# xarray-contrib/xeofs

Hardware: AMD Instinct MI355X
Metric: EOF randomized-SVD GB/s (algorithmic: 16 passes x n x p x 4 B per fit / fit time) (higher is better)
Workload: dtype f32 data, split-fp16 MFMA (f16x3+f16x3), f32 accumulate

## Files before the change

xeofs_amd/csrc/eofx_abi.hip:

```cpp
#include <chrono>
#include "eofx_hfft.hpp"
#include "eofx_kernels.hpp"
#include "eofx_fit.hpp"
#include "eofx_gram.hpp"
#include "eofx_axb_dma.hpp"
#include "eofx_hosteig.hpp"
#include "eofx_lag.hpp"
#include "eofx_gw.hpp"
#include "eofx_spca.hpp"
#include "eofx_lagcov.hpp"
#ifndef EOFX_AXB_DMA_DEFAULT
#define EOFX_AXB_DMA_DEFAULT 1
#endif

#if !defined(__HIP_DEVICE_COMPILE__)
#include <immintrin.h>
#endif
#include <algorithm>
#include <array>
#include <atomic>
#include <cmath>
#include <complex>
#include <cstdarg>
#include <cstdio>
// ... 880 lines not shown
        hipLaunchKernelGGL((axb_f16_dma_kernel<2, 0, true>), dim3(gx, 1), dim3(256), 0, ctx->stream, raw, ld, (int)rows, cols, aff,
                           aff_ld, ctx->axb_planes, pairs_all, out, L, rows_pad, K, plan.kps, plan.S, rt, nfull * 64, a_scale, bmax, act);
      else
        hipLaunchKernelGGL((axb_f16_dma_kernel<2, 0, false>), dim3(gx, 1), dim3(256), 0, ctx->stream, raw, ld, (int)rows, cols, aff,
                           aff_ld, ctx->axb_planes, pairs_all, out, L, rows_pad, K, plan.kps, plan.S, rt, nfull * 64, a_scale, bmax,
                           (const int*)nullptr);
      KCHK();
    }
  } else if (nfull > 0) {
    if (masked)
      hipLaunchKernelGGL((axb_f16_kernel<4, 0, true>), dim3(gx, nfull), dim3(256), 0, ctx->stream, raw, ld, (int)rows, cols, aff, aff_ld, Y,
                         L, out, L, rows_pad, K, plan.kps, plan.S, rt, 0, a_scale, bmax, act);
    else
      hipLaunchKernelGGL(axb_f16_kernel<4>, dim3(gx, nfull), dim3(256), 0, ctx->stream, raw, ld, (int)rows, cols, aff, aff_ld, Y, L, out,
                         L, rows_pad, K, plan.kps, plan.S, rt, 0, a_scale, bmax);
    KCHK();
  }
  if (!dma && rem) {
    if (masked)
      hipLaunchKernelGGL((axb_f16_kernel<2, 0, true>), dim3(gx, 1), dim3(256), 0, ctx->stream, raw, ld, (int)rows, cols, aff, aff_ld, Y, L,
                         out, L, rows_pad, K, plan.kps, plan.S, rt, nfull * 64, a_scale, bmax, act);
    else
      hipLaunchKernelGGL(axb_f16_kernel<2>, dim3(gx, 1), dim3(256), 0, ctx->stream, raw, ld, (int)rows, cols, aff, aff_ld, Y, L, out,
                         L, rows_pad, K, plan.kps, plan.S, rt, nfull * 64, a_scale, bmax);
    KCHK();
  }
  if (ctx->profile) {
    HIPCHK(hipEventRecord(ev1, ctx->stream));
    ctx->prof_events.emplace_back(ev0, ev1, 1);
    ctx->prof_flops += 2.0 * (double)K * (double)rows_pad * (double)L;
    ctx->prof_bytes += (double)K * (double)rows * 4.0 * (nfull + (rem ? 1 : 0));
  }
  if (plan.S > 1) {
    const int64_t count4 = rows_pad * L / 4;
    hipLaunchKernelGGL(splitk_reduce_kernel, dim3((int)std::min<int64_t>((count4 + 255) / 256, amax_out ? 2048 : 4096)), dim3(256), 0,
                       ctx->stream, out, W, count4, plan.S, amax_out);
    KCHK();
  }
  return EOFX_OK;
}

static int gram_parts(int64_t rows, int L) {
  const int64_t by_rows = std::min<int64_t>((rows + 127) / 128, 256);
  const int64_t by_mem = ((int64_t)128 << 20) / ((int64_t)L * L * 8);
  if (const char* ev = std::getenv("EOFX_GRAM_PARTS")) return std::max(1, atoi(ev));
  return (int)std::max<int64_t>(1, std::min(by_rows, std::max<int64_t>(by_mem, 1)));
}

static int launch_gram(eofx_ctx* ctx, const float* P, int64_t rows, int L, double* G) {
  const int nb = (L + 63) / 64;
  const int nbx = gram_parts(rows, L);
  ArenaScope scope(ctx);
  ARENA(double, part, (size_t)nbx * L * L);
  hipLaunchKernelGGL(gram_mfma_kernel, dim3(nbx, nb * nb), dim3(256), 0, ctx->stream, P, rows, L, part);
  KCHK();
  const int64_t count = (int64_t)L * L;
  hipLaunchKernelGGL(f64_reduce_kernel, dim3((int)((count + 63) / 64)), dim3(256), 0, ctx->stream,
                     part, G, count, nbx);
  KCHK();
  return EOFX_OK;
}
static int launch_matmul(eofx_ctx* ctx, const float* P, int64_t rows, int L, const double* Mx, int Lo,
                         float* out, bool upper = false) {
  int KW = (int)std::min<int64_t>(round_up(L, 64), 256);
  if (L > 256) {
    static const int kw_env = std::getenv("EOFX_PMM_KW") ? atoi(std::getenv("EOFX_PMM_KW")) : 0;
    if (kw_env == 128 || kw_env == 256) KW = kw_env;
  }
  const size_t smem = (size_t)KW * PMM_LD * sizeof(double);
  if (smem > 64 * 1024)
    HIPCHK(hipFuncSetAttribute(reinterpret_cast<const void*>(panel_matmul_kernel<false>), hipFuncAttributeMaxDynamicSharedMemorySize, (int)smem));
  const int64_t units = (rows + 127) / 128;
  const int64_t gx = L <= KW ? std::min<int64_t>(units, 1024) : units;
  dim3 grid((int)std::max<int64_t>(1, gx), (Lo + 63) / 64);
  hipLaunchKernelGGL(panel_matmul_kernel<false>, grid, dim3(256), smem, ctx->stream, P, rows, L, Mx, Lo, out, KW, amax_new(ctx, out),
                     (int64_t)0, (int64_t)0, 1, (const float*)nullptr, upper ? 1 : 0);
  KCHK();
  return EOFX_OK;
}
static int launch_matmul_gen(eofx_ctx* ctx, const float* P, int64_t ldp, int64_t slab, int cpb, int64_t rows, int L, const double* Mx, int Lo,
                             const float* sub, float* out) {
  const int KW = (int)std::min<int64_t>(round_up(L, 64), 256);
  const size_t smem = (size_t)KW * PMM_LD * sizeof(double);
  if (smem > 64 * 1024)
    HIPCHK(hipFuncSetAttribute(reinterpret_cast<const void*>(panel_matmul_kernel<true>), hipFuncAttributeMaxDynamicSharedMemorySize, (int)smem));
  const int64_t units = (rows + 127) / 128;
  const int64_t gx = L <= KW ? std::min<int64_t>(units, 1024) : units;
  dim3 grid((int)std::max<int64_t>(1, gx), (Lo + 63) / 64);
  hipLaunchKernelGGL(panel_matmul_kernel<true>, grid, dim3(256), smem, ctx->stream, P, rows, L, Mx, Lo, out, KW, amax_new(ctx, out), ldp,
                     slab, cpb, sub);
  KCHK();
  return EOFX_OK;
}
static int launch_xgram(eofx_ctx* ctx, const float* Pa, int64_t lda, int La, const float* Pb, int64_t ldb, int Lb, int64_t rows, double* C) {
  const int nbx = (int)std::max<int64_t>(1, std::min<int64_t>((rows + 127) / 128, std::max<int64_t>(1, ((int64_t)32 << 20) / ((int64_t)La * Lb * 8))));
  ArenaScope scope(ctx);
  ARENA(double, part, (size_t)nbx * La * Lb);
  hipLaunchKernelGGL(xgram_mfma_kernel, dim3(nbx, (La / 64) * (Lb / 64)), dim3(256), 0, ctx->stream, Pa, lda, Pb, ldb, rows, La, Lb, part);
  KCHK();
  const int64_t count = (int64_t)La * Lb;
  hipLaunchKernelGGL(f64_reduce_kernel, dim3((int)((count + 63) / 64)), dim3(256), 0, ctx->stream, part, C, count, nbx);
  KCHK();
  return EOFX_OK;
}

static void host_chol_rinv(const double* G, int L, int l, double* Rinv, double tol) {
  std::vector<double> A((size_t)l * l, 0.0), X((size_t)l * l, 0.0), d0(l);
// ... 9 lines not shown
    const double rjj = dj ? 1.0 : std::sqrt(d);
    const double piv = dj ? 0.0 : 1.0 / rjj;
    A[(size_t)j * l + j] = rjj;
    double* rowj = &A[(size_t)j * l];
    for (int c = j + 1; c < l; ++c) rowj[c] *= piv;
    for (int r = j + 1; r < l; ++r) {
      const double f = rowj[r];
      if (f == 0.0) continue;
      double* rowr = &A[(size_t)r * l];
      for (int c = r; c < l; ++c) rowr[c] -= f * rowj[c];
    }
  }
  for (int c = 0; c < l; ++c) {
    if (dead[c]) continue;
    X[(size_t)c * l + c] = 1.0 / A[(size_t)c * l + c];
    for (int r = c - 1; r >= 0; --r) {
      double sum = 0.0;
      for (int t = r + 1; t <= c; ++t) sum += A[(size_t)r * l + t] * X[(size_t)t * l + c];
      X[(size_t)r * l + c] = -sum / A[(size_t)r * l + r];
    }
  }
  for (int r = 0; r < L; ++r)
    for (int c = 0; c < L; ++c) Rinv[(size_t)r * L + c] = (r < l && c < l) ? X[(size_t)r * l + c] : 0.0;
}

static int launch_rinv(eofx_ctx* ctx, const double* G, int L, int l, double* Rinv);
static size_t rinv_blocked_bytes(int l);
static bool matmul_nt_ok(int64_t rows, int L, int Lo);
static size_t matmul_nt_scratch(eofx_ctx* ctx, int64_t rows, int L, int Lo);
static int launch_matmul_nt(eofx_ctx* ctx, const float* P, int64_t rows, int L, const double* Mx, int Lo, float* out);
static int launch_cholqr(eofx_ctx* ctx, const float* P, int64_t rows, int L, int l, const double* G,
                         float* out) {
  ArenaScope scope(ctx);
  ARENA(double, Rinv, (size_t)L * L);
  CHK(launch_rinv(ctx, G, L, l, Rinv));
  return launch_matmul(ctx, P, rows, L, Rinv, L, out, true);
}

static int launch_colminmax(eofx_ctx* ctx, const float* P, int64_t rows, int L, float* mx, float* mn) {
  const int nparts = (int)std::max<int64_t>(1, std::min<int64_t>((rows + 127) / 128, 1024));
  ArenaScope scope(ctx);
  ARENA(float, pmx, (size_t)nparts * L);
  ARENA(float, pmn, (size_t)nparts * L);
  hipLaunchKernelGGL(colminmax_part_kernel, dim3(nparts, (L + 63) / 64), dim3(256), 0, ctx->stream, P,
                     rows, L, pmx, pmn);
  KCHK();
  hipLaunchKernelGGL(colminmax_final_kernel, dim3((L + 63) / 64), dim3(256), 0, ctx->stream, pmx, pmn,
                     nparts, L, mx, mn);
  KCHK();
  return EOFX_OK;
}

static int export_panel(eofx_ctx* ctx, const float* P, int64_t rows, int L, int k, const double* sign,
                        float* dst) {
  if (!dst) return EOFX_OK;
  ArenaScope scope(ctx);
  double* dsign = nullptr;
  if (sign) {
    dsign = arena_alloc<double>(ctx, k);
    if (!dsign) return set_err(ctx, EOFX_ERR_NOMEM, "arena exhausted (export sign)");
    CHK(copy_in(ctx, dsign, sign, sizeof(double) * k));
  }
  float* tmp = dst;
  const bool dev = is_device_ptr(dst);
  if (!dev) {
    tmp = arena_alloc<float>(ctx, (size_t)rows * k);
    if (!tmp) return set_err(ctx, EOFX_ERR_NOMEM, "arena exhausted (export staging)");
  }
  const int64_t total = rows * k;
  const int blocks = (int)std::min<int64_t>((total + 255) / 256, 8192);
  hipLaunchKernelGGL(panel_export_kernel, dim3(blocks), dim3(256), 0, ctx->stream, P, rows, L, k, dsign,
                     tmp);
  KCHK();
  if (!dev) {
    CHK(copy_out(ctx, dst, tmp, sizeof(float) * total));
    HIPCHK(hipStreamSynchronize(ctx->stream));
  }
  return EOFX_OK;
}

static int import_panel(eofx_ctx* ctx, const float* src, int64_t rows, int l, float* P, int64_t rows_pad,
                        int L) {
  ArenaScope scope(ctx);
  const float* dsrc = src;
  if (!is_device_ptr(src)) {
    float* tmp = arena_alloc<float>(ctx, (size_t)rows * l);
    if (!tmp) return set_err(ctx, EOFX_ERR_NOMEM, "arena exhausted (import staging)");
    CHK(copy_in(ctx, tmp, src, sizeof(float) * rows * l));
    dsrc = tmp;
  }
  const int64_t total = rows_pad * (L / 4);
  const int blocks = (int)std::min<int64_t>((total + 255) / 256, 2048);
  hipLaunchKernelGGL(panel_import_kernel, dim3(blocks), dim3(256), 0, ctx->stream, dsrc, rows, l, P,
                     rows_pad, L, amax_new(ctx, P));
  KCHK();
  if (dsrc != src) HIPCHK(hipStreamSynchronize(ctx->stream));
  return EOFX_OK;
}

static void* pool_take(eofx_ctx* ctx, size_t bytes) {
  for (size_t i = 0; i < ctx->pool.size(); ++i)
    if (ctx->pool[i].second == bytes) {
      void* p = ctx->pool[i].first;
      ctx->pool_bytes -= bytes;
      ctx->pool.erase(ctx->pool.begin() + i);
      return p;
    }
  return nullptr;
}
static void pool_trim(eofx_ctx* ctx) {
  if (ctx->pool.empty()) return;
// ... 912 lines not shown
        int64_t off = 0;
        for (size_t i = 0; i < npairs; ++i) {
          const int m1 = 64 * seg[2 * i], m2 = 64 * seg[2 * i + 1];
          merge(off, m1, m2, 1, 0);
          KCHK();
          off += m1 + m2;
          next.push_back(seg[2 * i] + seg[2 * i + 1]);
        }
      }
      if (seg.size() & 1) next.push_back(seg.back());
      seg.swap(next);
    }
  }
  hipLaunchKernelGGL(chol_blocked_export_kernel, dim3(512), dim3(256), 0, ctx->stream, (const double*)X, Lb, l, Rinv, L);
  KCHK();
  return EOFX_OK;
}
static int launch_rinv(eofx_ctx* ctx, const double* G, int L, int l, double* Rinv) {
  if (l <= 64) {
    hipLaunchKernelGGL(chol_rinv_kernel, dim3(1), dim3(256), 0, ctx->stream, G, L, l, Rinv, 1e-13, (const double*)nullptr);
    KCHK();
  } else if (ctx->arena_size - ctx->arena_off >= rinv_blocked_bytes(l) && !std::getenv("EOFX_HOST_RINV")) {
    CHK(launch_rinv_blocked(ctx, G, L, l, Rinv));
  } else {
    std::vector<double> hG((size_t)L * L), hR((size_t)L * L);
    HIPCHK(hipMemcpyAsync(hG.data(), G, sizeof(double) * L * L, hipMemcpyDeviceToHost, ctx->stream));
    HIPCHK(hipStreamSynchronize(ctx->stream));
    host_chol_rinv(hG.data(), L, l, hR.data(), 1e-13);
    HIPCHK(hipMemcpyAsync(Rinv, hR.data(), sizeof(double) * L * L, hipMemcpyHostToDevice, ctx->stream));
    HIPCHK(hipStreamSynchronize(ctx->stream));
  }
  return EOFX_OK;
}

constexpr int EOFX_FIT_FALLBACK = 1;
typedef std::function<int(const float*, float*, int)> FirstFwd;
typedef std::function<int(const float*, float*, int)> RangeFinder;
static int rsvd_core(eofx_ctx* ctx, const LinOp& op, int k, int l, int n_iter, const float* omega,
                     RsvdOut& out, const FirstFwd* first_fwd = nullptr, const RangeFinder* range = nullptr) {
  const int L = (int)round_up(l, 32);
  const int Lo = (int)round_up(k, 32);
  AmaxScope amax_scope(ctx);
  ARENA(float, Zs, (size_t)op.small_pad * L);
  ARENA(float, Ws, (size_t)op.small_pad * L);
  ARENA(float, Yt, (size_t)op.tall_pad * L);
  ARENA(float, Qt, (size_t)op.tall_pad * L);
  ARENA(float, Tv, (size_t)op.tall_pad * Lo);
  ARENA(float, Sv, (size_t)op.small_pad * Lo);
  ARENA(double, G, (size_t)L * L);
  ARENA(double, G0, (size_t)L * L);
  ARENA(double, R2, (size_t)L * L);
  ARENA(double, Md, (size_t)L * Lo);
  ARENA(double, Md2, (size_t)L * Lo);
  double* pin = nullptr;
  CHK(pinned_scratch(ctx, &pin));
  if ((size_t)2 * L * L > EOFX_PINNED_DOUBLES) return set_err(ctx, EOFX_ERR_ARG, "internal: sketch too wide for the host scratch");

  CHK(import_panel(ctx, omega, op.small, l, Zs, op.small_pad, L));
  bool first_done = false;
  auto fwd = [&](const float* z, float* y, int prec) -> int {
    if (first_fwd && !first_done) {
      first_done = true;
      return (*first_fwd)(z, y, L);
    }
    first_done = true;
    return op.fwd(z, y, L, prec);
  };
  auto gram_tall = [&](const float* Pn, double* Gout) -> int {
    CHK(launch_gram(ctx, Pn, op.tall_pad, L, Gout));
    return op.reduce_tall_gram ? op.reduce_tall_gram(Gout, (int64_t)L * L) : EOFX_OK;
  };
  auto gram_small = [&](const float* Pn, double* Gout) -> int {
    CHK(launch_gram(ctx, Pn, op.small_pad, L, Gout));
    return op.reduce_small_gram ? op.reduce_small_gram(Gout, (int64_t)L * L) : EOFX_OK;
  };
  const int pp = ctx->prec_power, pf = ctx->prec_final;
  const bool orth_always = orth_tall_rule(op.rule_tall_pad > 0 ? op.rule_tall_pad : op.tall_pad, L, pp);
  bool orth_rest = orth_always;
  hipEvent_t peaked_ev = nullptr;
  bool peaked_pending = false;
  int rc = EOFX_OK;
  for (int it = 0; it < (range ? 0 : n_iter) && rc == EOFX_OK; ++it) {
    rc = fwd(Zs, Yt, pp);
    if (rc != EOFX_OK) break;
    if (peaked_pending) {
      peaked_pending = false;
      if (hipEventSynchronize(peaked_ev) != hipSuccess) rc = set_err(ctx, EOFX_ERR_HIP, "event wait failed");
      else orth_rest = eofx_peaked_spectrum(pin, L, l) != 0;
      if (rc != EOFX_OK) break;
    }
    if (it == 0 || orth_rest) {
      if ((rc = gram_tall(Yt, G)) != EOFX_OK) break;
      if ((rc = launch_cholqr(ctx, Yt, op.tall_pad, L, l, G, Qt)) != EOFX_OK) break;
      rc = op.bwd(Qt, Ws, L, pp);
    } else {
      rc = op.bwd(Yt, Ws, L, pp);
    }
    if (rc != EOFX_OK) break;
    const bool ask = it == 0 && !orth_always && n_iter > 1;
    if ((rc = gram_small(Ws, ask ? G0 : G)) != EOFX_OK) break;
    if (ask) {
      if (hipMemcpyAsync(pin, G0, sizeof(double) * L * L, hipMemcpyDeviceToHost, ctx->stream) != hipSuccess ||
          (!peaked_ev && hipEventCreateWithFlags(&peaked_ev, hipEventDisableTiming) != hipSuccess) ||
          hipEventRecord(peaked_ev, ctx->stream) != hipSuccess) {
        rc = set_err(ctx, EOFX_ERR_HIP, "asynchronous Gram download failed");
        break;
      }
      peaked_pending = true;
    }
    rc = launch_cholqr(ctx, Ws, op.small_pad, L, l, ask ? G0 : G, Zs);
  }
  if (peaked_ev) {
    if (peaked_pending) (void)hipEventSynchronize(peaked_ev);
    (void)hipEventDestroy(peaked_ev);
  }
  if (rc != EOFX_OK) return rc;
  if (range) CHK((*range)(Zs, Yt, L));
  else CHK(fwd(Zs, Yt, pp));
  CHK(gram_tall(Yt, G));
  CHK(launch_cholqr(ctx, Yt, op.tall_pad, L, l, G, Qt));
  CHK(gram_tall(Qt, G));
  CHK(launch_rinv(ctx, G, L, l, R2));
  CHK(op.bwd(Qt, Zs, L, pf));
  CHK(launch_matmul(ctx, Zs, op.small_pad, L, R2, L, Ws));
  CHK(gram_small(Ws, G));
  double* hG = pin;
  double* hR2 = pin + (size_t)L * L;
  HIPCHK(hipMemcpyAsync(hG, G, sizeof(double) * L * L, hipMemcpyDeviceToHost, ctx->stream));
  HIPCHK(hipMemcpyAsync(hR2, R2, sizeof(double) * L * L, hipMemcpyDeviceToHost, ctx->stream));
  HIPCHK(hipStreamSynchronize(ctx->stream));
  std::vector<double> Gl((size_t)l * l), w(l), Uh((size_t)l * l);
  for (int i = 0; i < l; ++i)
    for (int j = 0; j < l; ++j) {
      const double v = 0.5 * (hG[(size_t)i * L + j] + hG[(size_t)j * L + i]);
      if (!std::isfinite(v))
        return set_err(ctx, EOFX_ERR_LINALG,
                       "SVD failed. This may be due to isolated NaN values in the data.");
      Gl[(size_t)i * l + j] = v;
    }
  eofx_host_eigh_f64(Gl.data(), l, w.data(), Uh.data());
  out.s.assign(k, 0.0);
  std::vector<double> M1((size_t)L * Lo, 0.0), M2((size_t)L * Lo, 0.0);
  std::vector<double> invs(k);
  for (int j = 0; j < k; ++j) {
    const double sv = std::sqrt(std::max(w[j], 0.0));
    out.s[j] = sv;
    invs[j] = sv > 0.0 ? 1.0 / sv : 0.0;
  }
  for (int i = 0; i < l; ++i) {
    double* m1 = &M1[(size_t)i * Lo];
    for (int q = 0; q < l; ++q) {
      const double r = hR2[(size_t)i * L + q];
      const double* uq = &Uh[(size_t)q * l];
      for (int j = 0; j < k; ++j) m1[j] += r * uq[j];
    }
    for (int j = 0; j < k; ++j) M2[(size_t)i * Lo + j] = Uh[(size_t)i * l + j] * invs[j];
  }
  HIPCHK(hipMemcpyAsync(Md, M1.data(), sizeof(double) * L * Lo, hipMemcpyHostToDevice, ctx->stream));
  HIPCHK(hipMemcpyAsync(Md2, M2.data(), sizeof(double) * L * Lo, hipMemcpyHostToDevice, ctx->stream));
  CHK(launch_matmul(ctx, Qt, op.tall_pad, L, Md, Lo, Tv));
  CHK(launch_matmul(ctx, Ws, op.small_pad, L, Md2, Lo, Sv));
  HIPCHK(hipStreamSynchronize(ctx->stream));
  out.Tvec = Tv;
  out.Svec = Sv;
  out.Lo = Lo;
  out.tall_pad = op.tall_pad;
  out.small_pad = op.small_pad;
  return EOFX_OK;
}

static size_t rsvd_scratch_bytes(int64_t tall_pad, int64_t small_pad, int l, int k) {
  const size_t L = (size_t)round_up(l, 32), Lo = (size_t)round_up(k, 32);
  size_t b = 0;
  b += 2 * small_pad * L * 4 + 2 * tall_pad * L * 4 + tall_pad * Lo * 4 + small_pad * Lo * 4;
  b += atb_scratch_bytes(small_pad, tall_pad, (int)L);
  b += atb_scratch_bytes(tall_pad, small_pad, (int)L);
  b += atb_scratch_bytes(small_pad, tall_pad, (int)Lo);
  b += (size_t)(4 * gram_parts(std::max(tall_pad, small_pad), (int)L) + 8) * L * L * 8 + 2 * L * Lo * 8 + 4096;
  b += (size_t)std::max(tall_pad, small_pad) * (Lo + L) * 4;
  if (l > 64) b += rinv_blocked_bytes(l);
  b += 4 << 20;
  return b;
}

static int comm_allreduce(eofx_ctx* ctx, void* buf, int64_t count, int dtype, int op);
static int sign_rule(eofx_ctx* ctx, const float* Vpanel, int64_t rows, int Lo, int k,
                     std::vector<double>& sign, bool over_ranks = false) {
  ArenaScope scope(ctx);
  ARENA(float, mx, 2 * (size_t)Lo);
  float* mn = mx + Lo;
  CHK(launch_colminmax(ctx, Vpanel, rows, Lo, mx, mn));
  if (over_ranks) {
    hipLaunchKernelGGL(negate_kernel, dim3(1), dim3(256), 0, ctx->stream, mn, Lo);
    KCHK();
    CHK(comm_allreduce(ctx, mx, 2 * (int64_t)Lo, 0, 1));
    hipLaunchKernelGGL(negate_kernel, dim3(1), dim3(256), 0, ctx->stream, mn, Lo);
    KCHK();
  }
  std::vector<float> hmx(Lo), hmn(Lo);
  HIPCHK(hipMemcpyAsync(hmx.data(), mx, sizeof(float) * Lo, hipMemcpyDeviceToHost, ctx->stream));
  HIPCHK(hipMemcpyAsync(hmn.data(), mn, sizeof(float) * Lo, hipMemcpyDeviceToHost, ctx->stream));
  HIPCHK(hipStreamSynchronize(ctx->stream));
  sign.assign(k, 1.0);
  for (int j = 0; j < k; ++j) sign[j] = (std::fabs(hmx[j]) >= std::fabs(hmn[j])) ? 1.0 : -1.0;
  return EOFX_OK;
}

typedef std::function<int(double*, int64_t)> GramReduce;
static int fix_null_columns(eofx_ctx* ctx, float* P, int64_t rows, int64_t rows_pad, int Lo, int k, int first,
                            const GramReduce* reduce = nullptr, int64_t rows_total = -1) {
  if (rows_total < 0) rows_total = rows;
  if (first >= k || rows_total <= first) return EOFX_OK;
  if (!reduce) {
    const size_t need = (size_t)rows_pad * Lo * 4 + (size_t)(gram_parts(rows_pad, Lo) + 4) * Lo * Lo * 8 + (64 << 10);
    if (ctx->arena_size - ctx->arena_off < need) return EOFX_OK;
  }
  ArenaScope scope(ctx);
  ARENA(double, G, (size_t)Lo * Lo);
  ARENA(double, Mx, (size_t)Lo * Lo);
  ARENA(float, tmp, (size_t)rows_pad * Lo);
  ARENA(int, dflag, Lo);
  const int m = k - first;
  std::vector<double> hG((size_t)Lo * Lo), hM((size_t)Lo * Lo);
  std::vector<int> flag(Lo, 0);
  const int blocks = (int)std::max<int64_t>(1, std::min<int64_t>((rows + 255) / 256, 4096));
  auto gram = [&]() -> int {
    CHK(launch_gram(ctx, P, rows_pad, Lo, G));
    if (reduce && *reduce) CHK((*reduce)(G, (int64_t)Lo * Lo));
    HIPCHK(hipMemcpyAsync(hG.data(), G, sizeof(double) * Lo * Lo, hipMemcpyDeviceToHost, ctx->stream));
    HIPCHK(hipStreamSynchronize(ctx->stream));
    return EOFX_OK;
// ... 47 lines not shown
      }
    }
    if (dependent) {
      if (rounds_done > 0) break;
      CHK(refill());
      continue;
    }
    for (int c = 0; c < m; ++c) {
      Ri[(size_t)c * m + c] = 1.0 / A[(size_t)c * m + c];
      for (int r = c - 1; r >= 0; --r) {
        double sum = 0.0;
        for (int t = r + 1; t <= c; ++t) sum += A[(size_t)r * m + t] * Ri[(size_t)t * m + c];
        Ri[(size_t)r * m + c] = -sum / A[(size_t)r * m + r];
      }
    }
    std::fill(hM.begin(), hM.end(), 0.0);
    for (int i = 0; i < first; ++i) hM[(size_t)i * Lo + i] = 1.0;
    for (int a = 0; a < m; ++a)
      for (int b = a; b < m; ++b) hM[(size_t)(first + a) * Lo + first + b] = Ri[(size_t)a * m + b];
    for (int g = 0; g < first; ++g)
      for (int b = 0; b < m; ++b) {
        double v = 0.0;
        for (int a = 0; a <= b; ++a) v += hG[(size_t)g * Lo + first + a] * Ri[(size_t)a * m + b];
        hM[(size_t)g * Lo + first + b] = -v;
      }
    HIPCHK(hipMemcpyAsync(Mx, hM.data(), sizeof(double) * Lo * Lo, hipMemcpyHostToDevice, ctx->stream));
    CHK(launch_matmul(ctx, P, rows_pad, Lo, Mx, Lo, tmp));
    HIPCHK(hipMemcpy2DAsync(P + first, sizeof(float) * Lo, tmp + first, sizeof(float) * Lo, sizeof(float) * (size_t)(k - first), (size_t)rows_pad,
                            hipMemcpyDeviceToDevice, ctx->stream));
    HIPCHK(hipStreamSynchronize(ctx->stream));
    ++rounds_done;
  }
  return EOFX_OK;
}

static int fix_null_modes(eofx_ctx* ctx, const RsvdOut& ro, int64_t tall, int64_t small, int k,
                          const GramReduce* reduce_tall = nullptr, int64_t tall_total = -1,
                          const GramReduce* reduce_small = nullptr, int64_t small_total = -1) {
  int first_null = k;
  const double s0 = ro.s.empty() ? 0.0 : ro.s[0];
  for (int j = k - 1; j >= 0 && !(ro.s[j] > 1e-5 * s0); --j) first_null = j;
  if (first_null < k && s0 >= 0.0 && std::isfinite(s0) && ro.tall_pad >= tall && ro.small_pad >= small) {
    CHK(fix_null_columns(ctx, ro.Tvec, tall, ro.tall_pad, ro.Lo, k, first_null, reduce_tall, tall_total));
    CHK(fix_null_columns(ctx, ro.Svec, small, ro.small_pad, ro.Lo, k, first_null, reduce_small, small_total));
  }
  return EOFX_OK;
}

static int rsvd_finish(eofx_ctx* ctx, const RsvdOut& ro, bool transposed, int64_t n, int64_t p, int k, int flip,
                       float* U, float* s, float* V) {
  CHK(fix_null_modes(ctx, ro, transposed ? p : n, transposed ? n : p, k));
  const float* Vp = transposed ? ro.Tvec : ro.Svec;
  const float* Up = transposed ? ro.Svec : ro.Tvec;
  std::vector<double> sign;
  if (flip) CHK(sign_rule(ctx, Vp, p, ro.Lo, k, sign));
  CHK(export_panel(ctx, Up, n, ro.Lo, k, flip ? sign.data() : nullptr, U));
  CHK(export_panel(ctx, Vp, p, ro.Lo, k, flip ? sign.data() : nullptr, V));
  if (s) {
    std::vector<float> hs(k);
    for (int j = 0; j < k; ++j) hs[j] = (float)ro.s[j];
    HIPCHK(hipMemcpy(s, hs.data(), sizeof(float) * k, hipMemcpyDefault));
  }
  HIPCHK(hipStreamSynchronize(ctx->stream));
  return EOFX_OK;
}

extern "C" int eofx_rsvd_f32(eofx_ctx* ctx, const eofx_mat* m, int k, int n_oversamples, int n_iter,
                             const float* omega, int flip, float* U, float* s, float* V) {
  if (!ctx || !m || !omega || k <= 0 || n_oversamples < 0) return set_err(ctx, EOFX_ERR_ARG, "bad argument");
  ENTER(ctx);
  const int64_t n = m->n, p = m->p, r = std::min(n, p);
  if (k > r)
    return set_err(ctx, EOFX_ERR_RANK,
                   "n_modes must be less than or equal to the rank of the dataset (rank = %lld).", (long long)r);
  const int l_req = k + n_oversamples;
  const int l = (int)std::min<int64_t>(l_req, r);
  if (l > EOFX_MAX_SKETCH)
    return set_err(ctx, EOFX_ERR_ARG, "sketch width k+n_oversamples = %d > %d is not supported", l, EOFX_MAX_SKETCH);
  if (n_iter < 0) n_iter = rsvd_auto_iters(k, n, p);
  const bool transposed = n < p;
  LinOp op;
  if (transposed) {
    op = {p, n, m->p_pad, m->n_pad,
          [&](const float* z, float* y, int L, int pr) { return panel_tmul(ctx, m, z, y, L, pr); },
          [&](const float* y, float* w, int L, int pr) { return panel_mul(ctx, m, y, w, L, pr); }};
  } else {
    op = {n, p, m->n_pad, m->p_pad,
          [&](const float* z, float* y, int L, int pr) { return panel_mul(ctx, m, z, y, L, pr); },
          [&](const float* y, float* w, int L, int pr) { return panel_tmul(ctx, m, y, w, L, pr); }};
  }
  CHK(arena_reserve(ctx, rsvd_scratch_bytes(op.tall_pad, op.small_pad, l, k)));
  ArenaScope scope(ctx);
  std::vector<float> om_clamped;
  const float* om = omega;
  if (l == r) {
    om_clamped.assign((size_t)op.small * l, 0.f);
    for (int64_t i = 0; i < l; ++i) om_clamped[(size_t)i * l + i] = 1.f;
    om = om_clamped.data();
  } else if (l != l_req) {
    if (is_device_ptr(omega)) return set_err(ctx, EOFX_ERR_ARG, "omega must be a host pointer");
    om_clamped.resize((size_t)op.small * l);
    for (int64_t i = 0; i < op.small; ++i)
      for (int j = 0; j < l; ++j) om_clamped[(size_t)i * l + j] = omega[(size_t)i * l_req + j];
    om = om_clamped.data();
  }
  RsvdOut ro;
  CHK(rsvd_core(ctx, op, k, l, n_iter, om, ro));
  return rsvd_finish(ctx, ro, transposed, n, p, k, flip, U, s, V);
}

struct FitFirst {
  eofx_ctx* ctx = nullptr;
  const float* Xd = nullptr;
  int64_t n = 0, P = 0, p_pad = 0, n_pad = 0, K = 0;
// ... 3772 lines not shown
```

xeofs_amd/csrc/eofx_kernels.hpp:

```cpp
#pragma once
#include <hip/hip_runtime.h>
#include <stdint.h>

namespace eofx {

typedef float f32x16 __attribute__((ext_vector_type(16)));
typedef float f32x4 __attribute__((ext_vector_type(4)));
typedef float f32x2 __attribute__((ext_vector_type(2)));

__device__ __forceinline__ void aff_split(double sh, float& hi, float& lo) {
  hi = (float)sh;
  lo = (float)(sh - (double)hi);
}
__device__ __forceinline__ float aff_map(float x, float sh_hi, float sh_lo, float scale) {
  return ((x - sh_hi) - sh_lo) * scale;
}
__device__ __forceinline__ float aff_fma(float x, float sh_hi, float s, float nls) {
  return __builtin_fmaf(x - sh_hi, s, nls);
}

__device__ __forceinline__ void amax_commit(float mx, unsigned* __restrict__ amax_out) {
  __shared__ float amax_red_[16];
#pragma unroll
  for (int o = 32; o > 0; o >>= 1) mx = fmaxf(mx, __shfl_xor(mx, o));
// ... 958 lines not shown

__global__ __launch_bounds__(256) void gram_f64_kernel(const float* __restrict__ P, int64_t rows,
                                                        int L, double* __restrict__ Gpart) {
  __shared__ __attribute__((aligned(16))) float Pa[32][64];
  __shared__ __attribute__((aligned(16))) float Pb[32][64];
  const int nb = (L + 63) / 64;
  const int bi = blockIdx.y / nb, bj = blockIdx.y % nb;
  const int tid = threadIdx.x;
  const int ti = tid >> 4, tj = tid & 15;
  double acc[4][4];
#pragma unroll
  for (int x = 0; x < 4; ++x)
#pragma unroll
    for (int y = 0; y < 4; ++y) acc[x][y] = 0.0;
  const int lr = tid >> 4;
  const int lc = (tid & 15) * 4;
  for (int64_t r0 = (int64_t)blockIdx.x * 32; r0 < rows; r0 += (int64_t)gridDim.x * 32) {
#pragma unroll
    for (int h = 0; h < 2; ++h) {
      const int rr = lr + 16 * h;
      const int64_t r = r0 + rr;
      f32x4 va = {0.f, 0.f, 0.f, 0.f}, vb = {0.f, 0.f, 0.f, 0.f};
      if (r < rows) {
        const int ca = bi * 64 + lc, cb = bj * 64 + lc;
        if (ca < L) va = *reinterpret_cast<const f32x4*>(P + r * L + ca);
        if (cb < L) vb = *reinterpret_cast<const f32x4*>(P + r * L + cb);
      }
      *reinterpret_cast<f32x4*>(&Pa[rr][lc]) = va;
      *reinterpret_cast<f32x4*>(&Pb[rr][lc]) = vb;
    }
    __syncthreads();
#pragma unroll 8
    for (int r = 0; r < 32; ++r) {
      const f32x4 a = *reinterpret_cast<const f32x4*>(&Pa[r][4 * ti]);
      const f32x4 b = *reinterpret_cast<const f32x4*>(&Pb[r][4 * tj]);
#pragma unroll
      for (int x = 0; x < 4; ++x)
#pragma unroll
        for (int y = 0; y < 4; ++y) acc[x][y] += (double)a[x] * (double)b[y];
    }
    __syncthreads();
  }
  double* G = Gpart + (int64_t)blockIdx.x * L * L;
#pragma unroll
  for (int x = 0; x < 4; ++x)
#pragma unroll
    for (int y = 0; y < 4; ++y) {
      const int gi = bi * 64 + 4 * ti + x, gj = bj * 64 + 4 * tj + y;
      if (gi < L && gj < L) G[(int64_t)gi * L + gj] = acc[x][y];
    }
}


__global__ __launch_bounds__(256) void gram_mfma_kernel(const float* __restrict__ P, int64_t rows, int L,
                                                         double* __restrict__ Gpart) {
  const int nb = (L + 63) / 64;
  const int bi = blockIdx.y / nb, bj = blockIdx.y % nb;
  if (bi > bj) return;
  const int lane = threadIdx.x & 63, wave = threadIdx.x >> 6;
  const int lc = lane & 15, lk = lane >> 4;
  const int ca = 64 * bi + 4 * lc, cb = 64 * bj + 4 * lc;
  const bool same = (bi == bj);
  f64x4 acc[4][4];
#pragma unroll
  for (int x = 0; x < 4; ++x)
#pragma unroll
    for (int y = 0; y < 4; ++y) acc[x][y] = f64x4{0.0, 0.0, 0.0, 0.0};
  const int64_t wstride = (int64_t)gridDim.x * 4 * 4;
  auto fetch = [&](int64_t r0, f32x4& va, f32x4& vb) {
    const int64_t r = r0 + lk;
    va = f32x4{0.f, 0.f, 0.f, 0.f};
    vb = va;
    if (r < rows) {
      if (ca < L) va = *reinterpret_cast<const f32x4*>(P + r * L + ca);
      if (!same && cb < L) vb = *reinterpret_cast<const f32x4*>(P + r * L + cb);
    }
    if (same) vb = va;
  };
  constexpr int GRAM_PF = 4;
  int64_t r0 = ((int64_t)blockIdx.x * 4 + wave) * 4;
  f32x4 pa[GRAM_PF], pb[GRAM_PF];
#pragma unroll
  for (int d = 0; d < GRAM_PF; ++d) fetch(r0 + d * wstride, pa[d], pb[d]);
  for (; r0 < rows; r0 += GRAM_PF * wstride) {
#pragma unroll
    for (int d = 0; d < GRAM_PF; ++d) {
      const f32x4 va = pa[d], vb = pb[d];
      fetch(r0 + (GRAM_PF + d) * wstride, pa[d], pb[d]);
      __builtin_amdgcn_sched_barrier(0);
      if (same) {
#pragma unroll
        for (int x = 0; x < 4; ++x)
#pragma unroll
          for (int y = x; y < 4; ++y)
            acc[x][y] = __builtin_amdgcn_mfma_f64_16x16x4f64((double)va[x], (double)vb[y], acc[x][y], 0, 0, 0);
      } else {
#pragma unroll
        for (int x = 0; x < 4; ++x)
#pragma unroll
          for (int y = 0; y < 4; ++y)
            acc[x][y] = __builtin_amdgcn_mfma_f64_16x16x4f64((double)va[x], (double)vb[y], acc[x][y], 0, 0, 0);
      }
    }
  }
  __shared__ double Gs[64][65];
  for (int w = 0; w < 4; ++w) {
    if (wave == w) {
#pragma unroll
      for (int x = 0; x < 4; ++x)
#pragma unroll
        for (int y = 0; y < 4; ++y) {
          if (same && x > y) continue;
#pragma unroll
          for (int q = 0; q < 4; ++q) {
            const int i = 4 * (lk + 4 * q) + x, j = 4 * lc + y;
            if (w == 0) {
              Gs[i][j] = acc[x][y][q];
              if (same && x < y) Gs[j][i] = acc[x][y][q];
            } else {
              Gs[i][j] += acc[x][y][q];
              if (same && x < y) Gs[j][i] += acc[x][y][q];
            }
          }
        }
    }
    __syncthreads();
  }
  double* G = Gpart + (int64_t)blockIdx.x * (int64_t)L * L;
  for (int e = threadIdx.x; e < 64 * 64; e += 256) {
    const int i = e >> 6, j = e & 63;
    const int gi = 64 * bi + i, gj = 64 * bj + j;
    if (gi < L && gj < L) {
      G[(int64_t)gi * L + gj] = Gs[i][j];
      if (!same) G[(int64_t)gj * L + gi] = Gs[i][j];
    }
  }
}

__global__ __launch_bounds__(256) void f64_reduce_kernel(const double* __restrict__ part,
                                                         double* __restrict__ out, int64_t count,
                                                         int nparts) {
  __shared__ double red[4][64];
// ... 439 lines not shown
        for (int e = 0; e < 4; ++e) {
          mx[e] = fmaxf(mx[e], v[u][e]);
          mn[e] = fminf(mn[e], v[u][e]);
        }
    }
    for (; r < rows; r += step) {
      const f32x4 v = *reinterpret_cast<const f32x4*>(P + r * L + c);
#pragma unroll
      for (int e = 0; e < 4; ++e) {
        mx[e] = fmaxf(mx[e], v[e]);
        mn[e] = fminf(mn[e], v[e]);
      }
    }
  }
#pragma unroll
  for (int e = 0; e < 4; ++e) {
    smx[rl][4 * cq + e] = mx[e];
    smn[rl][4 * cq + e] = mn[e];
  }
  __syncthreads();
  if (tid < 64 && blockIdx.y * 64 + tid < L) {
    float a = smx[0][tid], b = smn[0][tid];
    for (int q = 1; q < 16; ++q) {
      a = fmaxf(a, smx[q][tid]);
      b = fminf(b, smn[q][tid]);
    }
    pmx[(int64_t)blockIdx.x * L + blockIdx.y * 64 + tid] = a;
    pmn[(int64_t)blockIdx.x * L + blockIdx.y * 64 + tid] = b;
  }
}
__global__ __launch_bounds__(256) void colminmax_final_kernel(const float* __restrict__ pmx,
                                                              const float* __restrict__ pmn, int nparts, int L,
                                                              float* __restrict__ mx, float* __restrict__ mn) {
  __shared__ float sa[4][64], sb[4][64];
  const int li = threadIdx.x & 63, qq = threadIdx.x >> 6;
  const int c = blockIdx.x * 64 + li;
  float a = -INFINITY, b = INFINITY;
  if (c < L) {
#pragma unroll 8
    for (int q = qq; q < nparts; q += 4) {
      a = fmaxf(a, pmx[(int64_t)q * L + c]);
      b = fminf(b, pmn[(int64_t)q * L + c]);
    }
  }
  sa[qq][li] = a;
  sb[qq][li] = b;
  __syncthreads();
  if (qq == 0 && c < L) {
    mx[c] = fmaxf(fmaxf(sa[0][li], sa[1][li]), fmaxf(sa[2][li], sa[3][li]));
    mn[c] = fminf(fminf(sb[0][li], sb[1][li]), fminf(sb[2][li], sb[3][li]));
  }
}

__global__ __launch_bounds__(256) void panel_export_kernel(const float* __restrict__ P,
                                                           int64_t rows, int L, int k,
                                                           const double* __restrict__ sign,
                                                           float* __restrict__ dst) {
  const int64_t total = rows * k;
  const int64_t stride = (int64_t)gridDim.x * blockDim.x;
  for (int64_t i = (int64_t)blockIdx.x * blockDim.x + threadIdx.x; i < total; i += stride) {
    const int64_t r = i / k;
    const int c = (int)(i - r * k);
    float v = P[r * L + c];
    if (sign) v *= (float)sign[c];
    dst[i] = v;
  }
}
__global__ __launch_bounds__(256) void panel_import_kernel(const float* __restrict__ src,
                                                           int64_t rows, int l,
                                                           float* __restrict__ P, int64_t rows_pad,
                                                           int L, unsigned* __restrict__ amax_out = nullptr) {
  const int l4 = L / 4;
  const int64_t total = rows_pad * l4;
  const int64_t stride = (int64_t)gridDim.x * blockDim.x;
  const bool small = total < ((int64_t)1 << 31);
  float mx = 0.f;
  for (int64_t i = (int64_t)blockIdx.x * blockDim.x + threadIdx.x; i < total; i += stride) {
    int64_t r;
    int c;
    if (small) {
      const unsigned iu = (unsigned)i, ru = iu / (unsigned)l4;
      r = ru;
      c = (int)(iu - ru * (unsigned)l4) * 4;
    } else {
      r = i / l4;
      c = (int)(i - r * l4) * 4;
    }
    f32x4 v = {0.f, 0.f, 0.f, 0.f};
    if (r < rows) {
      const float* sp = src + r * l + c;
#pragma unroll
      for (int e = 0; e < 4; ++e)
        if (c + e < l) v[e] = sp[e];
    }
    reinterpret_cast<f32x4*>(P)[i] = v;
    mx = fmaxf(mx, fmaxf(fmaxf(fabsf(v[0]), fabsf(v[1])), fmaxf(fabsf(v[2]), fabsf(v[3]))));
  }
  if (amax_out) amax_commit(mx, amax_out);
}

__global__ __launch_bounds__(256) void colstats_shift_kernel(const float* __restrict__ X, int64_t n, int64_t P, int64_t ld,
                                                              const int64_t* __restrict__ row_map, float* __restrict__ cshift) {
  const int64_t c = (int64_t)blockIdx.x * 256 + threadIdx.x;
  if (c >= P) return;
  float s = 0.f;
  for (int t = 0; t < 9; ++t) {
// ... 1036 lines not shown
```

Before: 5887.

## Move rotation build and sign rule to GPU, specialize narrow Gram kernel

Adds a single-column-block specialization of the f64 MFMA Gram kernel with a deeper prefetch, a uniform wave index and skipping of out-of-range rows. The host-side construction of the rotation matrices M1/M2 is replaced by a device kernel, so only the small eigenvector matrix and inverse singular values are uploaded, and the R2 download plus one stream sync are dropped. The sign rule now runs on the device via the column min/max kernels and a tiny sign kernel, so the sign vector never goes through the host. The final singular-value copy becomes async. Together these aim to remove host round-trips and host-side matrix products from the tail of the fit, at the cost of extra small kernel launches and a larger prefetch register footprint.

```diff
diff --git a/xeofs_amd/csrc/eofx_abi.hip b/xeofs_amd/csrc/eofx_abi.hip
--- a/xeofs_amd/csrc/eofx_abi.hip
+++ b/xeofs_amd/csrc/eofx_abi.hip
@@ -956,7 +956,8 @@
   const int nbx = gram_parts(rows, L);
   ArenaScope scope(ctx);
   ARENA(double, part, (size_t)nbx * L * L);
-  hipLaunchKernelGGL(gram_mfma_kernel, dim3(nbx, nb * nb), dim3(256), 0, ctx->stream, P, rows, L, part);
+  if (nb == 1) hipLaunchKernelGGL(gram_mfma_kernel<true>, dim3(nbx, 1), dim3(256), 0, ctx->stream, P, rows, L, part);
+  else hipLaunchKernelGGL(gram_mfma_kernel<false>, dim3(nbx, nb * nb), dim3(256), 0, ctx->stream, P, rows, L, part);
   KCHK();
   const int64_t count = (int64_t)L * L;
   hipLaunchKernelGGL(f64_reduce_kernel, dim3((int)((count + 63) / 64)), dim3(256), 0, ctx->stream,
@@ -1072,11 +1073,11 @@
 }
 
 static int export_panel(eofx_ctx* ctx, const float* P, int64_t rows, int L, int k, const double* sign,
-                        float* dst) {
+                        float* dst, bool sign_on_device = false) {
   if (!dst) return EOFX_OK;
   ArenaScope scope(ctx);
-  double* dsign = nullptr;
-  if (sign) {
+  double* dsign = sign_on_device ? const_cast<double*>(sign) : nullptr;
+  if (sign && !sign_on_device) {
     dsign = arena_alloc<double>(ctx, k);
     if (!dsign) return set_err(ctx, EOFX_ERR_NOMEM, "arena exhausted (export sign)");
     CHK(copy_in(ctx, dsign, sign, sizeof(double) * k));
@@ -2095,6 +2096,8 @@
   ARENA(double, R2, (size_t)L * L);
   ARENA(double, Md, (size_t)L * Lo);
   ARENA(double, Md2, (size_t)L * Lo);
+  ARENA(double, dUh, (size_t)L * L);
+  ARENA(double, dinvs, (size_t)Lo);
   double* pin = nullptr;
   CHK(pinned_scratch(ctx, &pin));
   if ((size_t)2 * L * L > EOFX_PINNED_DOUBLES) return set_err(ctx, EOFX_ERR_ARG, "internal: sketch too wide for the host scratch");
@@ -2168,11 +2171,9 @@
   CHK(launch_matmul(ctx, Zs, op.small_pad, L, R2, L, Ws));
   CHK(gram_small(Ws, G));
   double* hG = pin;
-  double* hR2 = pin + (size_t)L * L;
   HIPCHK(hipMemcpyAsync(hG, G, sizeof(double) * L * L, hipMemcpyDeviceToHost, ctx->stream));
-  HIPCHK(hipMemcpyAsync(hR2, R2, sizeof(double) * L * L, hipMemcpyDeviceToHost, ctx->stream));
   HIPCHK(hipStreamSynchronize(ctx->stream));
-  std::vector<double> Gl((size_t)l * l), w(l), Uh((size_t)l * l);
+  std::vector<double> Gl((size_t)l * l), w(l);
   for (int i = 0; i < l; ++i)
     for (int j = 0; j < l; ++j) {
       const double v = 0.5 * (hG[(size_t)i * L + j] + hG[(size_t)j * L + i]);
@@ -2181,29 +2182,22 @@
                        "SVD failed. This may be due to isolated NaN values in the data.");
       Gl[(size_t)i * l + j] = v;
     }
-  eofx_host_eigh_f64(Gl.data(), l, w.data(), Uh.data());
+  double* Uh = pin;
+  double* invs = pin + (size_t)L * L;
+  eofx_host_eigh_f64(Gl.data(), l, w.data(), Uh);
   out.s.assign(k, 0.0);
-  std::vector<double> M1((size_t)L * Lo, 0.0), M2((size_t)L * Lo, 0.0);
-  std::vector<double> invs(k);
   for (int j = 0; j < k; ++j) {
     const double sv = std::sqrt(std::max(w[j], 0.0));
     out.s[j] = sv;
     invs[j] = sv > 0.0 ? 1.0 / sv : 0.0;
   }
-  for (int i = 0; i < l; ++i) {
-    double* m1 = &M1[(size_t)i * Lo];
-    for (int q = 0; q < l; ++q) {
-      const double r = hR2[(size_t)i * L + q];
-      const double* uq = &Uh[(size_t)q * l];
-      for (int j = 0; j < k; ++j) m1[j] += r * uq[j];
-    }
-    for (int j = 0; j < k; ++j) M2[(size_t)i * Lo + j] = Uh[(size_t)i * l + j] * invs[j];
-  }
-  HIPCHK(hipMemcpyAsync(Md, M1.data(), sizeof(double) * L * Lo, hipMemcpyHostToDevice, ctx->stream));
-  HIPCHK(hipMemcpyAsync(Md2, M2.data(), sizeof(double) * L * Lo, hipMemcpyHostToDevice, ctx->stream));
+  HIPCHK(hipMemcpyAsync(dUh, Uh, sizeof(double) * l * l, hipMemcpyHostToDevice, ctx->stream));
+  HIPCHK(hipMemcpyAsync(dinvs, invs, sizeof(double) * k, hipMemcpyHostToDevice, ctx->stream));
+  hipLaunchKernelGGL(rot_build_kernel, dim3((L * Lo + 255) / 256), dim3(256), 0, ctx->stream, (const double*)R2, L, (const double*)dUh, l,
+                     (const double*)dinvs, k, Lo, Md, Md2);
+  KCHK();
   CHK(launch_matmul(ctx, Qt, op.tall_pad, L, Md, Lo, Tv));
   CHK(launch_matmul(ctx, Ws, op.small_pad, L, Md2, Lo, Sv));
-  HIPCHK(hipStreamSynchronize(ctx->stream));
   out.Tvec = Tv;
   out.Svec = Sv;
   out.Lo = Lo;
@@ -2219,7 +2213,7 @@
   b += atb_scratch_bytes(small_pad, tall_pad, (int)L);
   b += atb_scratch_bytes(tall_pad, small_pad, (int)L);
   b += atb_scratch_bytes(small_pad, tall_pad, (int)Lo);
-  b += (size_t)(4 * gram_parts(std::max(tall_pad, small_pad), (int)L) + 8) * L * L * 8 + 2 * L * Lo * 8 + 4096;
+  b += (size_t)(4 * gram_parts(std::max(tall_pad, small_pad), (int)L) + 9) * L * L * 8 + 3 * L * Lo * 8 + 4096;
   b += (size_t)std::max(tall_pad, small_pad) * (Lo + L) * 4;
   if (l > 64) b += rinv_blocked_bytes(l);
   b += 4 << 20;
@@ -2373,14 +2367,22 @@
   CHK(fix_null_modes(ctx, ro, transposed ? p : n, transposed ? n : p, k));
   const float* Vp = transposed ? ro.Tvec : ro.Svec;
   const float* Up = transposed ? ro.Svec : ro.Tvec;
-  std::vector<double> sign;
-  if (flip) CHK(sign_rule(ctx, Vp, p, ro.Lo, k, sign));
-  CHK(export_panel(ctx, Up, n, ro.Lo, k, flip ? sign.data() : nullptr, U));
-  CHK(export_panel(ctx, Vp, p, ro.Lo, k, flip ? sign.data() : nullptr, V));
+  ArenaScope scope(ctx);
+  double* dsign = nullptr;
+  if (flip) {
+    dsign = arena_alloc<double>(ctx, (size_t)ro.Lo);
+    float* mx = arena_alloc<float>(ctx, 2 * (size_t)ro.Lo);
+    if (!dsign || !mx) return set_err(ctx, EOFX_ERR_NOMEM, "arena exhausted (sign rule)");
+    CHK(launch_colminmax(ctx, Vp, p, ro.Lo, mx, mx + ro.Lo));
+    hipLaunchKernelGGL(sign_from_minmax_kernel, dim3(1), dim3(64), 0, ctx->stream, (const float*)mx, (const float*)(mx + ro.Lo), k, dsign);
+    KCHK();
+  }
+  CHK(export_panel(ctx, Up, n, ro.Lo, k, dsign, U, true));
+  CHK(export_panel(ctx, Vp, p, ro.Lo, k, dsign, V, true));
+  std::vector<float> hs(k);
   if (s) {
-    std::vector<float> hs(k);
     for (int j = 0; j < k; ++j) hs[j] = (float)ro.s[j];
-    HIPCHK(hipMemcpy(s, hs.data(), sizeof(float) * k, hipMemcpyDefault));
+    HIPCHK(hipMemcpyAsync(s, hs.data(), sizeof(float) * k, hipMemcpyDefault, ctx->stream));
   }
   HIPCHK(hipStreamSynchronize(ctx->stream));
   return EOFX_OK;
diff --git a/xeofs_amd/csrc/eofx_kernels.hpp b/xeofs_amd/csrc/eofx_kernels.hpp
--- a/xeofs_amd/csrc/eofx_kernels.hpp
+++ b/xeofs_amd/csrc/eofx_kernels.hpp
@@ -1034,15 +1034,16 @@
 }
 
 
+template <bool NARROW = false>
 __global__ __launch_bounds__(256) void gram_mfma_kernel(const float* __restrict__ P, int64_t rows, int L,
                                                          double* __restrict__ Gpart) {
-  const int nb = (L + 63) / 64;
-  const int bi = blockIdx.y / nb, bj = blockIdx.y % nb;
+  const int nb = NARROW ? 1 : (L + 63) / 64;
+  const int bi = NARROW ? 0 : blockIdx.y / nb, bj = NARROW ? 0 : blockIdx.y % nb;
   if (bi > bj) return;
-  const int lane = threadIdx.x & 63, wave = threadIdx.x >> 6;
+  const int lane = threadIdx.x & 63, wave = __builtin_amdgcn_readfirstlane(threadIdx.x >> 6);
   const int lc = lane & 15, lk = lane >> 4;
   const int ca = 64 * bi + 4 * lc, cb = 64 * bj + 4 * lc;
-  const bool same = (bi == bj);
+  const bool same = NARROW || (bi == bj);
   f64x4 acc[4][4];
 #pragma unroll
   for (int x = 0; x < 4; ++x)
@@ -1059,7 +1060,7 @@
     }
     if (same) vb = va;
   };
-  constexpr int GRAM_PF = 4;
+  constexpr int GRAM_PF = NARROW ? 16 : 4;
   int64_t r0 = ((int64_t)blockIdx.x * 4 + wave) * 4;
   f32x4 pa[GRAM_PF], pb[GRAM_PF];
 #pragma unroll
@@ -1067,9 +1068,10 @@
   for (; r0 < rows; r0 += GRAM_PF * wstride) {
 #pragma unroll
     for (int d = 0; d < GRAM_PF; ++d) {
-      const f32x4 va = pa[d], vb = pb[d];
+      const f32x4 va = pa[d], vb = NARROW ? pa[d] : pb[d];
       fetch(r0 + (GRAM_PF + d) * wstride, pa[d], pb[d]);
       __builtin_amdgcn_sched_barrier(0);
+      if (NARROW && r0 + d * wstride >= rows) continue;
       if (same) {
 #pragma unroll
         for (int x = 0; x < 4; ++x)
@@ -1615,6 +1617,26 @@
   }
 }
 
+__global__ __launch_bounds__(256) void rot_build_kernel(const double* __restrict__ R2, int L, const double* __restrict__ Uh,
+                                                        int l, const double* __restrict__ invs, int k, int Lo,
+                                                        double* __restrict__ M1, double* __restrict__ M2) {
+  for (int e = blockIdx.x * 256 + threadIdx.x; e < L * Lo; e += gridDim.x * 256) {
+    const int i = e / Lo, j = e % Lo;
+    double m1 = 0.0, m2 = 0.0;
+    if (i < l && j < k) {
+      for (int q = 0; q < l; ++q) m1 = __dadd_rn(m1, __dmul_rn(R2[(int64_t)i * L + q], Uh[q * l + j]));
+      m2 = __dmul_rn(Uh[i * l + j], invs[j]);
+    }
+    M1[e] = m1;
+    M2[e] = m2;
+  }
+}
+
+__global__ void sign_from_minmax_kernel(const float* __restrict__ mx, const float* __restrict__ mn, int k,
+                                        double* __restrict__ sign) {
+  for (int j = threadIdx.x; j < k; j += blockDim.x) sign[j] = (fabsf(mx[j]) >= fabsf(mn[j])) ? 1.0 : -1.0;
+}
+
 __global__ __launch_bounds__(256) void panel_export_kernel(const float* __restrict__ P,
                                                            int64_t rows, int L, int k,
                                                            const double* __restrict__ sign,
```

Result: no change. 5917, median of 6 (+0.5%).
